# agwi-lab/renderformer

Hardware: AMD Instinct MI355X
Metric: rendered frames/sec at 512×512, renderformer-v1.1-swin-large, 1/2/4/8 MI355X (higher is better)
Workload: dtype fp16+bf16

## Files before the change

renderformer_amd/csrc/gemm.hip:

```cpp
#include <algorithm>
#include <type_traits>
#include <cmath>
#include <math.h>
#include <stdio.h>
#include <stdlib.h>
#include <string.h>

#include "common.h"
#include "env.h"

namespace {

constexpr int BK = 32;
constexpr int P_F16 = 2;

enum Epi { E_BF16 = RF_EPI_BF16, E_F32 = RF_EPI_F32, E_ADD = RF_EPI_ADD_F32, E_SWIGLU = RF_EPI_SWIGLU, E_CONV = 16,
           E_ROPE = 17 };

template <int BM_, int BN_, int WGM_, int WGN_, int STAGES_, int KH_ = 1>
struct Tile {
    static constexpr int BM = BM_, BN = BN_, WGM = WGM_, WGN = WGN_, STAGES = STAGES_, KH = KH_;
    static constexpr int NWAVE = WGM * WGN, THREADS = NWAVE * 64;
    static constexpr int MW = BM / WGM, NWD = BN / WGN, TI = MW / 16, TJ = NWD / 16;
    static constexpr int APIECES = BM / 16;
    static constexpr bool ASHARE = APIECES < NWAVE;
    static constexpr int PA = ASHARE ? 1 : BM / 16 / NWAVE, PB = BN / 16 / NWAVE;
    static constexpr int A_BYTES = BM * BK * 2, B_BYTES = BN * BK * 2;
    static_assert(PA >= 1 && PB >= 1 && (ASHARE || PA * NWAVE * 16 == BM) && PB * NWAVE * 16 == BN,
                  "tile/wave mismatch");
    static_assert(TI >= 1 && TJ >= 2 && TJ % 2 == 0, "wave tile too small");
};

struct EngineArgs {
    const bf16_t* a;
    const bf16_t* a_lo;
    int64_t lda;
    const bf16_t* w;
    const bf16_t* w_lo;
    int64_t ldw;
    int m, n, k;
    int hi, wi, cin_pad, ho, wo, kw, stride, pad;
    uint64_t cin_m, kw_m;
    const bf16_t* zero;
    void* c;
    int64_t ldc;
    const float* bias;
    const float* res1;
    const float* res2;
    bf16_t* p_hi;
    bf16_t* p_lo;
    int p_ld;
    int cout, deconv, flags, n_fin;
    int plane_f16;
    const float* w_fin;
    const float* b_fin;
    float elu_alpha;
    float* sk_part;
    int* sk_flag;
    int sk_epoch;
    int group_m;
    const int* gate;
    int halo_lg;
    int* err;
    int spin;
    uint64_t* stamps;
    const uint8_t* sa;
    const uint8_t* sw;
    int ld_sa, ld_sw;
    int persist;
    int l2pf;
    int out_f16;
    int* range;
    bf16_t* xg;
    int64_t ldxg;
    const float* norm_g;
    float* ss_out;
    int xg_f16;
    const float* rs_part;
    float rs_n, rs_eps;
    float* seg_ss;
    int seg_w, seg_n;
// ... 253 lines not shown
            else if (younger >= 1) wait_vm<GB>();
            else wait_vm<0>();
        }
    };

#pragma unroll
    for (int s = 0; s < S; ++s)
        if (s < nk) issue(kbeg + s, s);
    wait_tile(std::min(S, nk) - 1);
    __builtin_amdgcn_s_barrier();
    __builtin_amdgcn_sched_barrier(0);
    Frags f0, f1;
    load_frags(0, f0);
    auto step = [&](int kt, Frags& cur, Frags& nxt) {
        __builtin_amdgcn_s_waitcnt(0xC07F);
        if (kt + 1 < nk) {
            const int y = std::min(S - 2, nk - 2 - kt);
            wait_tile(y < 0 ? 0 : y);
        }
        __builtin_amdgcn_s_barrier();
        __builtin_amdgcn_sched_barrier(0);
        if (kt + S < nk) issue(kbeg + kt + S, kt % S);
        if (kt + 1 < nk) load_frags(kt + 1, nxt);
        mma(cur);
    };
    for (int kt = 0; kt < nk; kt += 2) {
        step(kt, f0, f1);
        if (kt + 1 < nk) step(kt + 1, f1, f0);
    }
}

RF_DEV uint32_t lds_addr(const char* p) { return (uint32_t)(uintptr_t)LDS_PTR(const char, p); }
RF_DEV float lds_ld_f32(const char* p) {
    float v;
    asm volatile("ds_read_b32 %0, %1\n\ts_waitcnt lgkmcnt(0)" : "=v"(v) : "v"(lds_addr(p)) : "memory");
    return v;
}
RF_DEV f32x4 lds_ld_f4(const char* p) {
    f32x4 v;
    asm volatile("ds_read_b128 %0, %1\n\ts_waitcnt lgkmcnt(0)" : "=v"(v) : "v"(lds_addr(p)) : "memory");
    return v;
}
RF_DEV void lds_st_f32(char* p, float v) { asm volatile("ds_write_b32 %0, %1" ::"v"(lds_addr(p)), "v"(v) : "memory"); }
RF_DEV void lds_sync() {
    __builtin_amdgcn_sched_barrier(0);
    asm volatile("s_waitcnt lgkmcnt(0)" ::: "memory");
    __builtin_amdgcn_s_barrier();
    __builtin_amdgcn_sched_barrier(0);
}

template <class C>
constexpr int ROPE_POS_BYTES = (C::BM * 9 + 63) / 64 * 256;
template <class C, int EPI>
constexpr int PN_AREA = EPI == E_ADD      ? C::BN * 4 + C::BM * C::WGN * 4
                        : EPI == E_BF16   ? C::BM * PN_SLOTS * 4 + C::BM * C::WGN * 4
                        : EPI == E_ROPE   ? C::BM * PN_SLOTS * 4 + C::BM * C::WGN * 4 + C::BN * 4 + ROPE_POS_BYTES<C> + 64 * 4
                        : EPI == E_SWIGLU ? C::BM * PN_SLOTS * 4
                                          : 0;

template <class C, int EPI>
RF_DEV void pn_issue(const EngineArgs& p, char* area, int m0, int n0) {
    const int lane = threadIdx.x & 63;
    const int wave = __builtin_amdgcn_readfirstlane(threadIdx.x >> 6);
    if constexpr (EPI == E_ADD) {
        if (p.xg && wave == 0 && n0 + 4 * lane < p.n && 4 * lane < C::BN)
            __builtin_amdgcn_global_load_lds(GLB_PTR(void, p.norm_g + n0 + 4 * lane), LDS_PTR(void, area), 16, 0, 0);
    } else if constexpr (EPI == E_BF16 || EPI == E_SWIGLU || EPI == E_ROPE) {
        if (p.rs_part) {
            static_assert(C::BM % 32 == 0, "1-KiB pieces of 32 rows");
            for (int c = wave; c < C::BM / 32; c += C::NWAVE) {
                const int row = min(m0 + 32 * c + (lane >> 1), p.m - 1);
                __builtin_amdgcn_global_load_lds(GLB_PTR(void, p.rs_part + (int64_t)row * PN_SLOTS + 4 * (lane & 1)),
                                                 LDS_PTR(void, area + c * 1024), 16, 0, 0);
            }
        }
        if constexpr (EPI == E_ROPE) {
            if (n0 / p.seg_w < p.seg_n) {
                char* const gl = area + C::BM * PN_SLOTS * 4 + C::BM * C::WGN * 4;
                char* const pl = gl + C::BN * 4;
                char* const fl = pl + ROPE_POS_BYTES<C>;
                if (wave == 0 && p.rope_g && 4 * lane < C::BN)
                    __builtin_amdgcn_global_load_lds(GLB_PTR(void, p.rope_g + n0 + 4 * lane), LDS_PTR(void, gl), 16, 0, 0);
                if (p.rope_pos) {
                    if (wave == C::NWAVE - 1)
                        __builtin_amdgcn_global_load_lds(GLB_PTR(void, p.rope_freqs + min(lane, p.rope_nf - 1)),
                                                         LDS_PTR(void, fl), 4, 0, 0);
                    for (int c = wave; c * 64 < C::BM * 9; c += C::NWAVE) {
                        const int e = c * 64 + lane;
                        const int r = e / 9, col = e - r * 9;
                        const int row = min(m0 + min(r, C::BM - 1), p.m - 1) / p.rope_div;
                        __builtin_amdgcn_global_load_lds(GLB_PTR(void, p.rope_pos + (int64_t)row * p.rope_ld + col),
                                                         LDS_PTR(void, pl + c * 256), 4, 0, 0);
                    }
                }
            }
        }
    }
}

template <class C, int EPI, int TW2D = 0, bool FINAL = true>
RF_DEV void engine_epilogue(const EngineArgs& p, int m0, int n0, const f32x4 (&acc)[C::TI][C::TJ],
                            char* area = nullptr) {
    constexpr int TI = C::TI, TJ = C::TJ;
    const int lane = threadIdx.x & 63;
    const int wave = threadIdx.x >> 6;
    const int wm = wave / C::WGN, wn = wave % C::WGN;
    static_assert(TW2D == 0 || (EPI == E_CONV && TW2D % 16 == 0 && C::MW % TW2D == 0), "2-D conv tile");
    const int rl = lane & 15, cq = 4 * (lane >> 4);
    const int rbase = m0 + wm * C::MW, cbase = n0 + wn * C::NWD;
    auto frow = [&](int i) -> int {
        if constexpr (TW2D == 0) return rbase + i * 16 + rl;
        else return m0 + (wm * (C::MW / TW2D) + (i * 16) / TW2D) * p.wo + (i * 16) % TW2D + rl;
    };
    float amax = 0.f;
    const bool rsc = (EPI == E_SWIGLU || EPI == E_BF16 || EPI == E_ROPE) && p.rs_part && area;
    if constexpr (EPI == E_SWIGLU || EPI == E_BF16 || EPI == E_ROPE) {
        if (rsc) {
            lds_sync();
            for (int t = threadIdx.x; t < C::BM; t += C::THREADS) {
                char* q = area + t * (PN_SLOTS * 4);
                const f32x4 a = lds_ld_f4(q), b = lds_ld_f4(q + 16);
                const float sum = ((a[0] + a[1]) + (a[2] + a[3])) + ((b[0] + b[1]) + (b[2] + b[3]));
                lds_st_f32(q, 1.0f / sqrtf(sum / p.rs_n + p.rs_eps));
            }
            lds_sync();
        }
    }
    auto row_scale = [&](int i) -> float {
        return rsc ? lds_ld_f32(area + (wm * C::MW + i * 16 + rl) * (PN_SLOTS * 4)) : 1.f;
    };
    if constexpr (EPI == E_SWIGLU) {
// ... 133 lines not shown
            const PixOp& o = ops[PF ? (i & 1) : 0];
            if (frow(i) >= p.m) continue;
#pragma unroll
            for (int j = 0; j < TJ; ++j) {
                const int col = cbase + j * 16 + cq;
                if (col >= nreal) continue;
                const int64_t pix = o.pix[j];
                const int co = o.co[j];
                const float bb[4] = {o.b[j].x, o.b[j].y, o.b[j].z, o.b[j].w};
                const float rr1[4] = {o.r1[j].x, o.r1[j].y, o.r1[j].z, o.r1[j].w};
                const float rr2[4] = {o.r2[j].x, o.r2[j].y, o.r2[j].z, o.r2[j].w};
                float v[4] = {acc[i][j][0], acc[i][j][1], acc[i][j][2], acc[i][j][3]};
#pragma unroll
                for (int e = 0; e < 4; ++e) {
                    v[e] = ((v[e] + bb[e]) + rr1[e]) + rr2[e];
                    if (p.flags & RF_CONV_SILU_OUT) v[e] = silu(v[e]);
                }
                if (outp)
                    *reinterpret_cast<float4*>(outp + pix * p.cout + co) = make_float4(v[0], v[1], v[2], v[3]);
                if (p.p_hi && p.plane_f16) {
                    float a[4] = {v[0], v[1], v[2], v[3]};
                    if (p.flags & RF_CONV_PLANE_SILU) {
#pragma unroll
                        for (int e = 0; e < 4; ++e) a[e] = silu(a[e]);
                    }
                    amax = amax3(amax3(amax, a[0], a[1]), a[2], a[3]);
                    *reinterpret_cast<uint2*>(p.p_hi + pix * p.p_ld + co) = make_uint2(pack_f16x2(a[0], a[1]),
                                                                                       pack_f16x2(a[2], a[3]));
                } else if (p.p_hi) {
                    uint32_t h[2], l[2];
#pragma unroll
                    for (int e = 0; e < 2; ++e) {
                        float a0 = v[2 * e], a1 = v[2 * e + 1];
                        if (p.flags & RF_CONV_PLANE_SILU) {
                            a0 = silu(a0);
                            a1 = silu(a1);
                        }
                        const bf16_t h0 = f32_to_bf16(a0), h1 = f32_to_bf16(a1);
                        h[e] = (uint32_t)h0 | ((uint32_t)h1 << 16);
                        l[e] = pack_bf16x2(a0 - bf16_to_f32(h0), a1 - bf16_to_f32(h1));
                    }
                    *reinterpret_cast<uint2*>(p.p_hi + pix * p.p_ld + co) = make_uint2(h[0], h[1]);
                    *reinterpret_cast<uint2*>(p.p_lo + pix * p.p_ld + co) = make_uint2(l[0], l[1]);
                }
            }
        }
        if (p.range && !f16_in_range(amax)) report_f16_range(p.range, RF_RANGE_CONV);
        return;
    } else {
        const bool pre = EPI == E_ADD && p.xg && area;
        const bool qkseg = EPI == E_ROPE && n0 / p.seg_w < p.seg_n;
        const bool segq = (EPI == E_BF16 || (EPI == E_ROPE && qkseg)) && p.seg_ss && area && n0 / p.seg_w < p.seg_n;
        char* const red = area + (EPI == E_ADD ? C::BN * 4 : C::BM * PN_SLOTS * 4);
        if (pre) lds_sync();
        float ssr[TI];
#pragma unroll
        for (int i = 0; i < TI; ++i) ssr[i] = 0.f;
        const char* const gl = area + C::BM * PN_SLOTS * 4 + C::BM * C::WGN * 4;
        const float* const pl = reinterpret_cast<const float*>(gl + C::BN * 4);
        float frq[EPI == E_ROPE ? TJ : 1][2];
        int pcol[EPI == E_ROPE ? TJ : 1][2];
        float sscale = 1.f;
        if constexpr (EPI == E_ROPE) {
            if (qkseg) {
                if (!rsc) lds_sync();
                sscale = n0 / p.seg_w == 0 ? p.rope_qscale : 1.f;
                const int lim = 9 * p.rope_nf;
                const float* fl = pl + ROPE_POS_BYTES<C> / 4;
#pragma unroll
                for (int j = 0; j < TJ; ++j) {
                    const int col = cbase + j * 16 + cq;
#pragma unroll
                    for (int t = 0; t < 2; ++t) {
                        const int m = ((col & 127) >> 1) + t;
                        const bool on = p.rope_pos && m < lim;
                        const int pc = on ? m / p.rope_nf : 0;
                        frq[j][t] = on ? fl[m - pc * p.rope_nf] : 0.f;
                        pcol[j][t] = pc;
                    }
                }
            }
        }
#pragma unroll
        for (int i = 0; i < TI; ++i) {
            const int row = rbase + i * 16 + rl;
            if (row >= p.m) continue;
            const float rsi = row_scale(i);
#pragma unroll
            for (int j = 0; j < TJ; ++j) {
                const int col = cbase + j * 16 + cq;
                if (col >= p.n) continue;
                float v[4] = {acc[i][j][0] * rsi, acc[i][j][1] * rsi, acc[i][j][2] * rsi, acc[i][j][3] * rsi};
                if (p.bias) {
                    const float4 b = *reinterpret_cast<const float4*>(p.bias + col);
                    v[0] += b.x;
                    v[1] += b.y;
                    v[2] += b.z;
                    v[3] += b.w;
                }
                const int64_t o = (int64_t)row * p.ldc + col;
                if constexpr (EPI == E_ROPE) {
                    if (qkseg) {
                        if (segq) ssr[i] += v[0] * v[0] + v[1] * v[1] + v[2] * v[2] + v[3] * v[3];
                        const f32x4 g = p.rope_g ? *reinterpret_cast<const f32x4*>(gl + (col - n0) * 4)
                                                 : f32x4{1.f, 1.f, 1.f, 1.f};
                        const float z0 = v[0] * g[0], z1 = v[1] * g[1], z2 = v[2] * g[2], z3 = v[3] * g[3];
                        const float* prow = pl + (wm * C::MW + i * 16 + rl) * 9;
                        float s0, c0, s1, c1;
                        __sincosf(prow[pcol[j][0]] * frq[j][0], &s0, &c0);
                        __sincosf(prow[pcol[j][1]] * frq[j][1], &s1, &c1);
                        v[0] = (z0 * c0 - z1 * s0) * sscale;
                        v[1] = (z1 * c0 + z0 * s0) * sscale;
                        v[2] = (z2 * c1 - z3 * s1) * sscale;
                        v[3] = (z3 * c1 + z2 * s1) * sscale;
                    }
                    *reinterpret_cast<uint2*>(reinterpret_cast<bf16_t*>(p.c) + o) =
                        make_uint2(pack_bf16x2(v[0], v[1]), pack_bf16x2(v[2], v[3]));
                } else if constexpr (EPI == E_BF16) {
                    amax = amax3(amax3(amax, v[0], v[1]), v[2], v[3]);
                    const uint32_t lo = pack16(p, v[0], v[1]), hi = pack16(p, v[2], v[3]);
                    *reinterpret_cast<uint2*>(reinterpret_cast<bf16_t*>(p.c) + o) = make_uint2(lo, hi);
                    if (segq) {
                        const float r0 = unpack16(p, lo & 0xffffu), r1 = unpack16(p, lo >> 16);
                        const float r2 = unpack16(p, hi & 0xffffu), r3 = unpack16(p, hi >> 16);
                        ssr[i] += r0 * r0 + r1 * r1 + r2 * r2 + r3 * r3;
                    }
                } else {
                    *reinterpret_cast<float4*>(reinterpret_cast<float*>(p.c) + o) = make_float4(v[0], v[1], v[2], v[3]);
                    if (pre) {
                        const f32x4 g = lds_ld_f4(area + (col - n0) * 4);
                        const float y0 = v[0] * g[0], y1 = v[1] * g[1], y2 = v[2] * g[2], y3 = v[3] * g[3];
                        amax = amax3(amax3(amax, y0, y1), y2, y3);
                        const uint32_t lo = p.xg_f16 ? pack_f16x2(y0, y1) : pack_bf16x2(y0, y1);
                        const uint32_t hi = p.xg_f16 ? pack_f16x2(y2, y3) : pack_bf16x2(y2, y3);
                        *reinterpret_cast<uint2*>(p.xg + (int64_t)row * p.ldxg + col) = make_uint2(lo, hi);
                        ssr[i] += v[0] * v[0] + v[1] * v[1] + v[2] * v[2] + v[3] * v[3];
                    }
                }
            }
        }
        if constexpr (EPI == E_BF16)
            if (p.range && !f16_in_range(amax)) report_f16_range(p.range, RF_RANGE_GEMM);
        if constexpr (EPI == E_ADD || EPI == E_BF16 || EPI == E_ROPE) {
            if (pre && p.xg_f16 && p.range && !f16_in_range(amax)) report_f16_range(p.range, RF_RANGE_RMSNORM);
            if (pre || segq) {
#pragma unroll
                for (int i = 0; i < TI; ++i) {
                    ssr[i] += __shfl_xor(ssr[i], 16, 64);
                    ssr[i] += __shfl_xor(ssr[i], 32, 64);
                }
                if (lane < 16) {
#pragma unroll
                    for (int i = 0; i < TI; ++i) lds_st_f32(red + (wn * C::BM + wm * C::MW + i * 16 + rl) * 4, ssr[i]);
                }
                lds_sync();
                int slot, nslots, ld;
                float* base;
                if (pre) {
                    slot = n0 / C::BN;
                    nslots = (p.n + C::BN - 1) / C::BN;
                    ld = PN_SLOTS;
                    base = p.ss_out;
                } else {
                    slot = (n0 % p.seg_w) / C::BN;
                    nslots = p.seg_w / C::BN;
                    ld = p.seg_n * PN_SLOTS;
                    base = p.seg_ss + (n0 / p.seg_w) * PN_SLOTS;
                }
                for (int t = threadIdx.x; t < C::BM; t += C::THREADS) {
                    const int row = m0 + t;
                    if (row < p.m) {
                        float s = 0.f;
#pragma unroll
                        for (int w = 0; w < C::WGN; ++w) s += lds_ld_f32(red + (w * C::BM + t) * 4);
                        float* dst = base + (int64_t)row * ld;
                        dst[slot] = s;
                        if (slot == 0)
                            for (int z = nslots; z < PN_SLOTS; ++z) dst[z] = 0.f;
                    }
                }
            }
        }
    }
}



namespace ph {
constexpr int BN = 256, BK2 = 64;
constexpr int REGION = 16384;
template <int BM>
struct Cfg {
    static constexpr int NREG = BM == 256 ? 4 : 3;
    static constexpr int NA = BM == 256 ? 2 : 1;
    static constexpr int A_IMG = BM * 128;
    static constexpr int TILE = A_IMG + 256 * 128;
    static constexpr int LDS = 2 * TILE;
    static constexpr int MI = BM / 32;
    static constexpr int GLDS = 2 * NREG;
    static constexpr int FA = BM == 256 ? 4 : BM / 32;
    static_assert(BM == 256 || BM == 128 || BM == 96 || BM == 64, "phased tile height");
};
template <int BM>
RF_DEV int region_row(int r, int j) {
    if constexpr (BM == 256) {
        switch (r) {
            case 0: return j < 64 ? j : j + 64;
            case 1: return j < 64 ? j + 64 : j + 128;
            case 2: return (j >> 5) * 64 + (j & 31);
            default: return (j >> 5) * 64 + 32 + (j & 31);
        }
    } else {
        switch (r) {
            case 0: return j;
            case 1: return (j >> 5) * 64 + (j & 31);
            default: return (j >> 5) * 64 + 32 + (j & 31);
        }
    }
}
template <int ROWS>
RF_DEV int img(int row, int kh, int ch) { return kh * (ROWS * 64) + row * 64 + ((ch ^ ((row >> 1) & 3)) << 4); }
}

template <int BM, int NTERM, bool GATHER, bool INITC = false>
RF_DEV void phased_mainloop(const EngineArgs& p, char* smem, int m0, int n0, int kbeg, int kend,
                            f32x4 (&acc)[BM / 32][4], bool pre = false) {
    using namespace ph;
    using G = Cfg<BM>;
    constexpr int NREG = G::NREG, NA = G::NA, MI = G::MI;
    static_assert(NTERM == 1 || NTERM == P_F16, "phased loop: single-term operands");
    constexpr int FA = G::FA;
    const int lane = threadIdx.x & 63;
    const int wave = threadIdx.x >> 6;
    const int wr = wave >> 2, wc = wave & 3;
    const int nk = kend - kbeg;
    const bool has_a = BM >= 128 || __builtin_amdgcn_readfirstlane(wave) < BM / 16;

    const int jrow = 16 * wave + (lane >> 2);
    int trow[NREG], grow[NREG];
    const bf16_t* src[NREG];
#pragma unroll
    for (int r = 0; r < NREG; ++r) {
        trow[r] = region_row<BM>(r, jrow);
        grow[r] = region_row<BM>(r, 16 * wave);
    }
    int am[NA], gi[NA], gy[NA], gx[NA];
#pragma unroll
    for (int r = 0; r < NA; ++r) {
        const int m = m0 + trow[r];
        am[r] = m < p.m ? m : p.m - 1;
        src[r] = p.a + (int64_t)am[r] * p.lda;
        gi[r] = gy[r] = gx[r] = 0;
        if constexpr (GATHER) {
            const int ox = am[r] % p.wo, t = am[r] / p.wo;
            gi[r] = m < p.m ? t / p.ho : -1;
            gy[r] = (t % p.ho) * p.stride - p.pad;
            gx[r] = ox * p.stride - p.pad;
        }
    }
#pragma unroll
    for (int r = NA; r < NREG; ++r) src[r] = p.w + (int64_t)(n0 + trow[r]) * p.ldw;
    const int lch = lane & 3;

    auto issue = [&](int kt, int r) {
        const bool is_a = r < NA;
        if (is_a && !has_a) return;
        char* base = smem + (kt & 1) * G::TILE + (is_a ? 0 : G::A_IMG);
#pragma unroll
        for (int kh = 0; kh < 2; ++kh) {
            const int row = trow[r];
            const int ch = lch ^ ((row >> 1) & 3);
            const int k0 = (kbeg + kt) * BK2 + kh * 32;
            const bf16_t* g = src[r] + k0 + ch * 8;
            if constexpr (GATHER) {
                if (is_a) {
                    const int tap = udiv_m(k0, p.cin_m), cb = k0 - tap * p.cin_pad;
                    const int ky = udiv_m(tap, p.kw_m), kx = tap - ky * p.kw;
                    const int iy = gy[r] + ky, ix = gx[r] + kx;
                    const bool ok = gi[r] >= 0 && iy >= 0 && iy < p.hi && ix >= 0 && ix < p.wi;
                    g = ok ? p.a + (((int64_t)gi[r] * p.hi + iy) * p.wi + ix) * p.cin_pad + cb + ch * 8 : p.zero;
                }
            }
            char* dst = base + kh * (is_a ? BM * 64 : 256 * 64) + grow[r] * 64;
            __builtin_amdgcn_global_load_lds(GLB_PTR(void, g), LDS_PTR(void, dst), 16, 0, 0);
        }
    };

    if (INITC && kbeg == 0) {
        load_c_acc<MI, 4>(p, m0 + wr * (BM / 2), n0 + wc * 64, acc);
    } else {
#pragma unroll
        for (int i = 0; i < MI; ++i)
#pragma unroll
            for (int j = 0; j < 4; ++j) acc[i][j] = f32x4{0.f, 0.f, 0.f, 0.f};
    }

    const int frow = lane & 15, fch = lane >> 4;
    bf16x8 fa[FA][2], fb0[2][2], fb1[2][2];
    auto read_a = [&](const char* buf, int mi) {
#pragma unroll
        for (int i = 0; i < FA; ++i)
#pragma unroll
            for (int s = 0; s < 2; ++s)
                fa[i][s] = *reinterpret_cast<const bf16x8*>(buf + img<BM>(wr * (BM / 2) + mi * 64 + i * 16 + frow, s, fch));
    };
    auto read_b = [&](const char* buf, int ni, bf16x8 (&fb)[2][2]) {
#pragma unroll
        for (int j = 0; j < 2; ++j)
#pragma unroll
            for (int s = 0; s < 2; ++s)
                fb[j][s] = *reinterpret_cast<const bf16x8*>(buf + G::A_IMG + img<256>(wc * 64 + ni * 32 + j * 16 + frow, s, fch));
    };
    auto mma = [&](int mi, int ni, const bf16x8 (&fb)[2][2]) {
        __builtin_amdgcn_s_setprio(1);
#pragma unroll
        for (int s = 0; s < 2; ++s)
#pragma unroll
            for (int i = 0; i < FA; ++i)
#pragma unroll
                for (int j = 0; j < 2; ++j) {
                    f32x4& c = acc[mi * FA + i][ni * 2 + j];
                    if constexpr (NTERM == P_F16)
                        c = __builtin_amdgcn_mfma_f32_16x16x32_f16(__builtin_bit_cast(f16x8, fb[j][s]),
                                                                   __builtin_bit_cast(f16x8, fa[i][s]), c, 0, 0, 0);
                    else
                        c = __builtin_amdgcn_mfma_f32_16x16x32_bf16(fb[j][s], fa[i][s], c, 0, 0, 0);
                }
        __builtin_amdgcn_s_setprio(0);
    };
    auto sync_in = [&]() {
        __builtin_amdgcn_s_waitcnt(0xC07F);
        __builtin_amdgcn_sched_barrier(0);
        __builtin_amdgcn_s_barrier();
        __builtin_amdgcn_sched_barrier(0);
    };
    auto sync_out = [&]() {
        __builtin_amdgcn_sched_barrier(0);
        __builtin_amdgcn_s_barrier();
        __builtin_amdgcn_sched_barrier(0);
    };

    constexpr int AHEAD = BM == 256 ? 8 : 4;
    if (!pre) {
#pragma unroll
        for (int r = 0; r < NREG; ++r) issue(0, r);
    }
    if (nk > 1) {
        if (!pre) {
#pragma unroll
            for (int r = 0; r < (BM == 256 ? NREG : 2); ++r) issue(1, r);
        }
        if (has_a) wait_vm<AHEAD>();
        else wait_vm<AHEAD - 2>();
    } else {
        wait_vm<0>();
    }
    __builtin_amdgcn_s_barrier();
    __builtin_amdgcn_sched_barrier(0);
    const bool late = __builtin_amdgcn_readfirstlane(threadIdx.x) >= 256;
    if (late) __builtin_amdgcn_s_barrier();
    __builtin_amdgcn_sched_barrier(0);

    for (int t = 0; t < nk; ++t) {
        const char* buf = smem + (t & 1) * G::TILE;
        const bool pf = t + 2 < nk;
        if constexpr (BM == 256) {
            read_b(buf, 0, fb0);
            read_a(buf, 0);
            sync_in();
            mma(0, 0, fb0);
            sync_out();
            read_b(buf, 1, fb1);
            if (pf) {
                issue(t + 2, 0);
                issue(t + 2, 2);
            }
            sync_in();
            mma(0, 1, fb1);
            sync_out();
            read_a(buf, 1);
            if (pf) issue(t + 2, 3);
            sync_in();
            mma(1, 1, fb1);
            sync_out();
            if (pf) {
                issue(t + 2, 1);
                wait_vm<8>();
            } else {
                wait_vm<0>();
            }
            sync_in();
            mma(1, 0, fb0);
            sync_out();
        } else {
            read_b(buf, 0, fb0);
            read_a(buf, 0);
            if (t + 1 < nk) issue(t + 1, 2);
            sync_in();
            mma(0, 0, fb0);
            sync_out();
            read_b(buf, 1, fb1);
            if (pf) {
                issue(t + 2, 0);
                issue(t + 2, 1);
                if (has_a) wait_vm<4>();
                else wait_vm<2>();
            } else {
                wait_vm<0>();
            }
            sync_in();
            mma(0, 1, fb1);
            sync_out();
        }
    }
    if (!late) __builtin_amdgcn_s_barrier();
}

template <int BM, int NTERM, bool INITC>
RF_DEV void phased3_mainloop(const EngineArgs& p, char* smem, int m0, int n0, int kbeg, int kend,
                             f32x4 (&acc)[BM / 32][4], char* touch_lds = nullptr) {
    using namespace ph;
    using G = Cfg<BM>;
    static_assert(BM <= 128, "three-buffer loop: short tiles");
    constexpr int NREG = 3, FA = G::FA;
    const int lane = threadIdx.x & 63;
    const int wave = threadIdx.x >> 6;
    const int wr = wave >> 2, wc = wave & 3;
    const int nk = kend - kbeg;
    const bool has_a = BM >= 128 || __builtin_amdgcn_readfirstlane(wave) < BM / 16;
    const int jrow = 16 * wave + (lane >> 2);
    int trow[NREG], grow[NREG];
    const bf16_t* src[NREG];
#pragma unroll
    for (int r = 0; r < NREG; ++r) {
        trow[r] = region_row<BM>(r, jrow);
        grow[r] = region_row<BM>(r, 16 * wave);
    }
    {
        const int m = m0 + trow[0];
        src[0] = p.a + (int64_t)(m < p.m ? m : p.m - 1) * p.lda;
// ... 112 lines not shown
        sync_in();
        mma(0, fb0);
        sync_out();
        read_b(buf, 1, fb1);
        if (t + 2 < nk) {
            if (l2pf) {
                if (has_a) wait_vm<8>();
                else wait_vm<6>();
            } else {
                if (has_a) wait_vm<6>();
                else wait_vm<4>();
            }
        } else {
            wait_vm<0>();
        }
        sync_in();
        mma(1, fb1);
        sync_out();
    }
    if (!late) __builtin_amdgcn_s_barrier();
}

template <int BM, int EPI, int NTERM = 1>
__global__ __launch_bounds__(512, 1) void phased3_kernel(EngineArgs p) {
    using TE = Tile<BM, 256, 2, 4, 4>;
#ifdef RF_STUDY
    __shared__ __attribute__((aligned(16))) char smem[3 * ph::Cfg<BM>::TILE + PN_AREA<TE, EPI> + 256];
#else
    __shared__ __attribute__((aligned(16))) char smem[3 * ph::Cfg<BM>::TILE + PN_AREA<TE, EPI>];
#endif
    if (gated_off(p)) return;
    const int tiles_m = (p.m + BM - 1) / BM;
    const int nwg = gridDim.x;
    const int hw = blockIdx.x;
    const int xcd = hw & 7, q = nwg >> 3, r = nwg & 7;
    const int wg = (xcd < r ? xcd * (q + 1) : r * (q + 1) + (xcd - r) * q) + (hw >> 3);
    int tm, tn;
    tile_coords(wg, tiles_m, p.n / ph::BN, p.group_m, tm, tn);
    f32x4 acc[BM / 32][4];
    char* const area = smem + 3 * ph::Cfg<BM>::TILE;
    pn_issue<TE, EPI>(p, area, tm * BM, tn * ph::BN);
#ifdef RF_STUDY
    char* const touch = area + PN_AREA<TE, EPI>;
#else
    char* const touch = nullptr;
#endif
    phased3_mainloop<BM, NTERM, EPI == E_ADD>(p, smem, tm * BM, tn * ph::BN, 0, p.k / ph::BK2, acc, touch);
    engine_epilogue<TE, EPI>(p, tm * BM, tn * ph::BN, acc, area);
}

template <int BM, int EPI, int NTERM, bool GATHER>
__global__ __launch_bounds__(512, 1) void phased_kernel(EngineArgs p) {
    using TE = Tile<BM, 256, 2, 4, 4>;
    __shared__ __attribute__((aligned(16))) char smem[ph::Cfg<BM>::LDS + PN_AREA<TE, EPI>];
    if (gated_off(p)) return;
    const int tiles_m = (p.m + BM - 1) / BM;
    const int nwg = gridDim.x;
    const int hw = blockIdx.x;
    const int xcd = hw & 7, q = nwg >> 3, r = nwg & 7;
    const int wg = (xcd < r ? xcd * (q + 1) : r * (q + 1) + (xcd - r) * q) + (hw >> 3);
    int tm, tn;
    tile_coords(wg, tiles_m, p.n / ph::BN, p.group_m, tm, tn);
    f32x4 acc[BM / 32][4];
    char* const area = smem + ph::Cfg<BM>::LDS;
    pn_issue<TE, EPI>(p, area, tm * BM, tn * ph::BN);
    phased_mainloop<BM, NTERM, GATHER, EPI == E_ADD>(p, smem, tm * BM, tn * ph::BN, 0, p.k / ph::BK2, acc);
    engine_epilogue<TE, EPI>(p, tm * BM, tn * ph::BN, acc, area);
}

RF_DEV void phased_issue01(const EngineArgs& p, char* smem, int m0, int n0, int nk) {
    using namespace ph;
    using G = Cfg<256>;
    const int lane = threadIdx.x & 63, wave = threadIdx.x >> 6;
    const int jrow = 16 * wave + (lane >> 2), lch = lane & 3;
#pragma unroll
    for (int kt = 0; kt < 2; ++kt) {
        if (kt == 1 && nk < 2) break;
#pragma unroll
        for (int r = 0; r < G::NREG; ++r) {
            const bool is_a = r < G::NA;
            const int trow = region_row<256>(r, jrow), grow = region_row<256>(r, 16 * wave);
            const bf16_t* src;
            if (is_a) {
                const int m = m0 + trow;
                src = p.a + (int64_t)(m < p.m ? m : p.m - 1) * p.lda;
            } else {
                src = p.w + (int64_t)(n0 + trow) * p.ldw;
            }
            char* base = smem + (kt & 1) * G::TILE + (is_a ? 0 : G::A_IMG);
#pragma unroll
            for (int kh = 0; kh < 2; ++kh) {
                const int ch = lch ^ ((trow >> 1) & 3);
                const bf16_t* g = src + kt * BK2 + kh * 32 + ch * 8;
                char* dst = base + kh * (256 * 64) + grow * 64;
                __builtin_amdgcn_global_load_lds(GLB_PTR(void, g), LDS_PTR(void, dst), 16, 0, 0);
            }
        }
    }
}

template <int EPI, int NTERM>
__global__ __launch_bounds__(512, 1) void phased_sk_kernel(EngineArgs p) {
    constexpr int TI = 8, TJ = 4, BM = 256, TS = BM * ph::BN;
    using TE = Tile<256, 256, 2, 4, 4>;
    __shared__ __attribute__((aligned(16))) char smem[ph::Cfg<BM>::LDS + PN_AREA<TE, EPI>];
    char* const area = smem + ph::Cfg<BM>::LDS;
// ... 1460 lines not shown
    p.sk_part = (float*)workspace;
    p.sk_flag = (int*)(p.sk_part + SK_PART_FLOATS);
    p.sk_epoch = rf::next_epoch(p.sk_flag, SK_MAX_GRID * sizeof(int), (hipStream_t)stream);
    if (p.sk_epoch == 0) return RF_ERR_LAUNCH;
    p.err = rf::device_error_word();
    p.spin = rf::spin_limit();
    p.stamps = RF_ENV_ONCE("RF_GEMM_STAMPS", 0) != 0 ? (uint64_t*)(p.sk_part + SK_PART_FLOATS - 65536) : nullptr;
    return RF_OK;
}

template <class F>
int with_epi(int epilogue, F&& f) {
    switch (epilogue) {
        case RF_EPI_BF16: return f(std::integral_constant<int, E_BF16>{});
        case RF_EPI_F32: return f(std::integral_constant<int, E_F32>{});
        case RF_EPI_ADD_F32: return f(std::integral_constant<int, E_ADD>{});
        default: return f(std::integral_constant<int, E_SWIGLU>{});
    }
}

inline void dense_args(EngineArgs& p, const void* a, int64_t lda, const void* w, int64_t ldw, int m, int n, int k,
                       void* c, int64_t ldc) {
    p.a = (const bf16_t*)a;
    p.lda = lda;
    p.w = (const bf16_t*)w;
    p.ldw = ldw;
    p.m = m;
    p.n = n;
    p.k = k;
    p.c = c;
    p.ldc = ldc;
}


int sk_grid(int m, int n, int k) {
    const bool env = rf::env_set("RF_GEMM_SK");
    int grid = 2 * 256;
    if (!env) return 0;
    if (env) {
        grid = rf::env_int("RF_GEMM_SK", 0);
        if (grid <= 0) return 0;
        grid = grid > SK_MAX_GRID ? SK_MAX_GRID : grid;
    }
    const int64_t tiles = (int64_t)((m + 127) / 128) * (n / 128);
    const int64_t rounds = (tiles + 511) / 512;
    const double eff = (double)tiles / (rounds * 512);
    if (!env && (eff >= 0.9 || tiles * (k / BK) < 8LL * grid)) return 0;
    return grid;
}

enum TileCode : int {
    TC_R128 = 128,
    TC_P256 = 256,
    TC_R64 = 642,
    TC_P64 = 643,
    TC_R64w4 = 644,
    TC_P3_64 = 645,
    TC_R64s6 = 646,
    TC_R96 = 962,
    TC_P96 = 963,
    TC_P3_96 = 964,
    TC_R96s5 = 965,
    TC_R96s6 = 966,
    TC_P128 = 1282,
    TC_P3_128 = 1283,
    TC_R128s4 = 1284,
    TC_R128s5 = 1285,
    TC_R128s6 = 1286,
    TC_R128w8s6 = 1288,
    TC_R256x128 = 2561,
    TC_R64k2 = 6423,
    TC_R64w4k2 = 6443,
    TC_R96k2 = 9623,
    TC_R128k2s3 = 12823,
    TC_R128k2s4 = 12824,
    TC_R128w8k2 = 12884,
};

int pick_cfg(int m, int n, int k, int epilogue = RF_EPI_BF16) {
    if (rf::env_set("RF_GEMM_TILE")) return rf::env_int("RF_GEMM_TILE", 0);
    const bool phased = n % 256 == 0 && k % 64 == 0 && rf::env_int("RF_GEMM_PHASED", 1) != 0;
    const double kk = k / 1024.0;
    const bool add = epilogue == RF_EPI_ADD_F32;
    auto cost = [&](int bm, int bn, int slots, double fixed, double per_k, double add_cost) {
        const int64_t tiles = (int64_t)((m + bm - 1) / bm) * (n / bn);
        const int64_t rounds = (tiles + 256 * slots - 1) / (256 * slots);
        return rounds * (fixed + per_k * kk + (add ? add_cost : 0.0));
    };
    int best = TC_R128;
    const int64_t t128 = (int64_t)((m + 127) / 128) * (n / 128);
    double best_c = t128 <= 256 ? cost(128, 128, 1, 5.5, 13.1, 5.0) : cost(128, 128, 2, 11.0, 14.0, 5.0);
    auto consider = [&](int cfg, double c) {
        if (c < best_c) {
            best_c = c;
            best = cfg;
        }
    };
    if (k % 64 == 0) consider(TC_R128w8k2, cost(128, 128, 1, 6.8, 10.9, 5.0));
    if (n % 256 == 0) consider(TC_R96, cost(96, 256, 1, 2.2, 16.5, 13.0));
    if (phased) {
        consider(TC_P256, cost(256, 256, 1, 11.0, 20.4, 5.0));
        consider(TC_P128, cost(128, 256, 1, 2.3, 18.4, 5.0));
        consider(TC_P3_96, cost(96, 256, 1, 6.0, 14.4, 5.0));
        consider(TC_P3_64, cost(64, 256, 1, 6.5, 11.8, 5.0));
    }
    return best;
}

__device__ __attribute__((aligned(16))) bf16_t g_zero_row[64];

namespace mx {
constexpr int BM = 256, BN = 256, KS = 128;
constexpr int A_DATA = BM * KS, B_DATA = BN * KS;
constexpr int STAGE = A_DATA + B_DATA + (BM + BN) * 4;
constexpr int TI = 8, TJ = 4;
typedef __attribute__((ext_vector_type(8))) int i32x8;
RF_DEV int off(int row, int ch) { return row * KS + ((ch ^ (row & 7)) << 4); }
}

template <bool INITC>
RF_DEV void mx8_mainloop(const EngineArgs& p, char* smem, int m0, int n0, int kbeg, int kend,
                         f32x4 (&acc)[mx::TI][mx::TJ]) {
    using namespace mx;
    const int lane = threadIdx.x & 63;
    const int wave = threadIdx.x >> 6;
    const int wm = wave >> 2, wn = wave & 3;
    const int nk = kend - kbeg;
    const uint8_t* A = reinterpret_cast<const uint8_t*>(p.a);
    const uint8_t* W = reinterpret_cast<const uint8_t*>(p.w);
    auto issue = [&](int kt, int buf) {
        char* st = smem + buf * STAGE;
        const int64_t k0 = (int64_t)(kbeg + kt) * KS;
#pragma unroll
        for (int i = 0; i < 8; ++i) {
            const int piece = wave * 8 + i;
            const bool is_a = piece < BM / 8;
            const int row = (is_a ? piece : piece - BM / 8) * 8 + (lane >> 3);
            const int ch = (lane & 7) ^ (row & 7);
            const uint8_t* src;
            if (is_a) {
                const int m = m0 + row;
                src = A + (int64_t)(m < p.m ? m : p.m - 1) * p.lda + k0 + ch * 16;
            } else {
                src = W + (int64_t)(n0 + row) * p.ldw + k0 + ch * 16;
            }
            __builtin_amdgcn_global_load_lds(GLB_PTR(void, src), LDS_PTR(void, st + (is_a ? 0 : A_DATA) + piece % (BM / 8) * 1024),
                                             16, 0, 0);
        }
        {
            const bool is_a = wave < BM / 64;
            const int row = (is_a ? wave : wave - BM / 64) * 64 + lane;
            const uint8_t* src;
            if (is_a) {
                const int m = m0 + row;
// ... 289 lines not shown

#ifdef RF_STUDY
int l2pf_dist() {
    return std::max(0, std::min(8, rf::env_int("RF_GEMM_L2PF", 0)));
}
#endif

template <int EPI, int BM, int NT = 1>
int launch_phased3(EngineArgs a, void* stream, const char* what) {
#ifdef RF_STUDY
    a.l2pf = l2pf_dist();
#endif
    const int tiles_m = (a.m + BM - 1) / BM, tiles_n = a.n / 256;
    const int nwg = tiles_n * tiles_m;
    a.group_m = pick_group_m(tiles_m, tiles_n, BM, 256, (nwg + 7) / 8, (int64_t)a.m * a.k * 2);
    RF_LAUNCH((phased3_kernel<BM, EPI, NT>), dim3(nwg), dim3(512), 0, (hipStream_t)stream, a);
    return rf::check_launch(what);
}

template <int EPI, int NT = 1>
int launch_phased_sk(EngineArgs a, int grid, void* stream, const char* what) {
    const int tiles_m = (a.m + 255) / 256, tiles_n = a.n / 256;
    a.group_m = pick_group_m(tiles_m, tiles_n, 256, 256, ((int64_t)tiles_m * tiles_n + 7) / 8);
    RF_LAUNCH((phased_sk_kernel<EPI, NT>), dim3(grid), dim3(512), 0, (hipStream_t)stream, a);
    return rf::check_launch(what);
}

bool use_phased(int n, int k) {
    return rf::env_int("RF_GEMM_PHASED", 1) != 0 && n % 256 == 0 && k % 64 == 0;
}

template <class C>
struct Ring {};
template <int BM>
struct Phased {};
template <int BM>
struct Phased3 {};

enum Pre { PRE_NONE = 0, PRE_N256 = 1, PRE_K64 = 2, PRE_PHASED = 4 };

bool pre_ok(int pre, const EngineArgs& p) {
    return (!(pre & PRE_N256) || p.n % 256 == 0) && (!(pre & PRE_K64) || p.k % 64 == 0) &&
           (!(pre & PRE_PHASED) || use_phased(p.n, p.k));
}

template <int CODE, class LOOP, int PRE, bool F16>
struct Row {};
template <class... R>
struct Rows {};

using TileTable = Rows<
    Row<TC_P256,        Phased<256>,                      PRE_PHASED,          true>,
    Row<TC_P128,        Phased<128>,                      PRE_PHASED,          true>,
    Row<TC_P256,        Ring<T256>,                       PRE_N256,            false>,
    Row<TC_R128s4,      Ring<Tile<128, 128, 2, 2, 4>>,    PRE_NONE,            false>,
    Row<TC_R128s5,      Ring<Tile<128, 128, 2, 2, 5>>,    PRE_NONE,            false>,
    Row<TC_R256x128,    Ring<T256x128>,                   PRE_NONE,            false>,
    Row<TC_R96,         Ring<T96x256>,                    PRE_N256,            true>,
    Row<TC_R64,         Ring<T64x256>,                    PRE_N256,            false>,
    Row<TC_P3_128,      Phased3<128>,                     PRE_PHASED,          true>,
    Row<TC_P3_96,       Phased3<96>,                      PRE_PHASED,          true>,
    Row<TC_P3_64,       Phased3<64>,                      PRE_PHASED,          true>,
    Row<TC_P96,         Phased<96>,                       PRE_PHASED,          false>,
    Row<TC_P64,         Phased<64>,                       PRE_PHASED,          false>,
    Row<TC_R64w4,       Ring<T64x256w4>,                  PRE_N256,            false>,
    Row<TC_R96s5,       Ring<T96x256s5>,                  PRE_N256,            false>,
    Row<TC_R96s6,       Ring<T96x256s6>,                  PRE_N256,            false>,
    Row<TC_R64s6,       Ring<T64x256s6>,                  PRE_N256,            false>,
    Row<TC_R128s6,      Ring<T128s6>,                     PRE_NONE,            false>,
    Row<TC_R128w8s6,    Ring<T128w8s6>,                   PRE_NONE,            false>,
    Row<TC_R128k2s3,    Ring<T128k2s3>,                   PRE_K64,             false>,
    Row<TC_R128k2s4,    Ring<T128k2s4>,                   PRE_K64,             false>,
    Row<TC_R128w8k2,    Ring<T128w8k2s4>,                 PRE_K64,             true>,
    Row<TC_R96k2,       Ring<T96x256k2>,                  PRE_K64 | PRE_N256,  false>,
    Row<TC_R64k2,       Ring<T64x256k2>,                  PRE_K64 | PRE_N256,  false>,
    Row<TC_R64w4k2,     Ring<T64x256w4k2>,                PRE_K64 | PRE_N256,  false>,
    Row<TC_R128,        Ring<T128>,                       PRE_NONE,            true>>;

template <int NT, class C>
int run_loop(Ring<C>, const EngineArgs& p, int epilogue, void* stream) {
    return with_epi(epilogue, [&](auto e) { return launch<C, decltype(e)::value, NT>(p, stream, "rf_gemm"); });
}
template <int NT, int BM>
int run_loop(Phased<BM>, const EngineArgs& p, int epilogue, void* stream) {
    return with_epi(epilogue, [&](auto e) {
        return launch_phased<decltype(e)::value, NT, false, BM>(p, stream, NT == P_F16 ? "rf_gemm_f16" : "rf_gemm_bf16");
    });
}
template <int NT, int BM>
int run_loop(Phased3<BM>, const EngineArgs& p, int epilogue, void* stream) {
    return with_epi(epilogue, [&](auto e) { return launch_phased3<decltype(e)::value, BM, NT>(p, stream, "rf_gemm"); });
}

template <int NT, int CODE, class LOOP, int PRE, bool F16>
bool try_row(Row<CODE, LOOP, PRE, F16>, int cfg, const EngineArgs& p, int epilogue, void* stream, int& rc) {
    if constexpr (NT == P_F16 && !F16) {
        return false;
    } else {
        if (cfg != CODE || !pre_ok(PRE, p)) return false;
        rc = run_loop<NT>(LOOP{}, p, epilogue, stream);
        return true;
    }
}

template <int NT, class... R>
int run_dp(Rows<R...>, int cfg, const EngineArgs& p, int epilogue, void* stream) {
// ... 192 lines not shown
    nio.rs_n = (float)norm_dim;
    nio.rs_eps = eps;
    nio.seg_ss = seg_ss;
    nio.seg_w = seg_w;
    nio.seg_n = seg_ss ? n_seg : 0;
    return gemm_bf16(a, lda, w, ldw, c, ldc, nullptr, m, n, k, epilogue, workspace, ws_bytes, stream, nullptr,
                     operand_dtype == RF_DT_F16, &nio);
}

template <class C, int NT>
static int launch_rope(EngineArgs p, void* stream) {
    return launch<C, E_ROPE, NT>(p, stream, "rf_gemm_qk_rope");
}

extern "C" int rf_gemm_qk_rope(const void* a, int64_t lda, const void* w, int64_t ldw, void* c, int64_t ldc, int m,
                               int n, int k, const float* ss, int norm_dim, float eps, float* seg_ss, int seg_w,
                               int n_seg, const float* norm_w, const float* pos, int64_t ld_pos, int pos_div,
                               const float* freqs, int n_freqs, float q_scale, int operand_dtype, void* workspace,
                               int64_t ws_bytes, void* stream) {
    (void)workspace;
    (void)ws_bytes;
    RF_REQUIRE(a && w && c, "rf_gemm_qk_rope: null pointer");
    RF_REQUIRE(m > 0 && n > 0 && k > 0, "rf_gemm_qk_rope: empty problem m=%d n=%d k=%d", m, n, k);
    RF_REQUIRE(operand_dtype == RF_DT_F16 || operand_dtype == RF_DT_BF16, "rf_gemm_qk_rope: operand_dtype");
    RF_REQUIRE(k % 64 == 0 && n % 128 == 0, "rf_gemm_qk_rope: needs K %% 64 == 0 and N %% 128 == 0");
    RF_REQUIRE(lda % 8 == 0 && ldw % 8 == 0 && lda >= k && ldw >= k && ((uintptr_t)a & 15) == 0 &&
                   ((uintptr_t)w & 15) == 0, "rf_gemm_qk_rope: operands must be 16-B aligned with lda/ldw >= K");
    RF_REQUIRE(ldc >= n && ldc % 4 == 0 && ((uintptr_t)c & 7) == 0, "rf_gemm_qk_rope: ldc too small/unaligned");
    RF_REQUIRE(seg_w > 0 && seg_w % 256 == 0 && seg_w % 128 == 0 && n_seg >= 1 && (int64_t)seg_w * n_seg <= n,
               "rf_gemm_qk_rope: the q/k segments must be whole 256-column tiles inside N");
    RF_REQUIRE(!seg_ss || (((uintptr_t)seg_ss & 15) == 0 && seg_w <= PN_SLOTS * 128),
               "rf_gemm_qk_rope: seg_ss must be 16-B aligned and seg_w <= %d", PN_SLOTS * 128);
    RF_REQUIRE(!ss || (((uintptr_t)ss & 15) == 0 && norm_dim > 0), "rf_gemm_qk_rope: ss must be 16-B aligned");
    RF_REQUIRE(!norm_w || ((uintptr_t)norm_w & 15) == 0, "rf_gemm_qk_rope: norm_w must be 16-B aligned");
    RF_REQUIRE(!pos || (freqs && n_freqs > 0 && 9 * n_freqs <= 64 && ld_pos >= 9 && pos_div >= 1),
               "rf_gemm_qk_rope: pos needs freqs with 9 * n_freqs <= 64, ld_pos >= 9 and pos_div >= 1");
    EngineArgs p{};
    dense_args(p, a, lda, w, ldw, m, n, k, c, ldc);
    p.rs_part = ss;
    p.rs_n = (float)norm_dim;
    p.rs_eps = eps;
    p.seg_ss = norm_w ? seg_ss : nullptr;
    p.seg_w = seg_w;
    p.seg_n = n_seg;
    p.rope_pos = pos;
    p.rope_ld = ld_pos;
    p.rope_div = pos ? pos_div : 1;
    p.rope_freqs = freqs;
    p.rope_nf = pos ? n_freqs : 1;
    p.rope_g = norm_w;
    p.rope_qscale = q_scale;
    const bool f16 = operand_dtype == RF_DT_F16;
    const int cfg = pick_cfg(m, n, k, RF_EPI_BF16);
    const bool t96 = n % 256 == 0 && cfg != TC_R128w8k2;
    if (t96) return f16 ? launch_rope<T96x256, P_F16>(p, stream) : launch_rope<T96x256, 1>(p, stream);
    return f16 ? launch_rope<T128w8k2s4, P_F16>(p, stream) : launch_rope<T128w8k2s4, 1>(p, stream);
}

extern "C" int rf_gemm_bf16_if(const int* flag, const void* a, int64_t lda, const void* w, int64_t ldw, void* c,
                               int64_t ldc, const float* bias, int m, int n, int k, int epilogue, void* workspace,
                               int64_t ws_bytes, void* stream) {
    RF_REQUIRE(flag, "rf_gemm_bf16_if: null flag");
    return gemm_bf16(a, lda, w, ldw, c, ldc, bias, m, n, k, epilogue, workspace, ws_bytes, stream, flag);
}

extern "C" int rf_gemm_mx8(const void* a, int64_t lda, const void* sa, int64_t ld_sa, const void* w, int64_t ldw,
                           const void* sw, int64_t ld_sw, void* c, int64_t ldc, const float* bias, int m, int n, int k,
                           int epilogue, void* stream) {
    RF_REQUIRE(a && w && sa && sw && c, "rf_gemm_mx8: null pointer");
    RF_REQUIRE(m > 0 && n > 0 && k > 0, "rf_gemm_mx8: empty problem");
    RF_REQUIRE(k % 128 == 0 && n % 256 == 0, "rf_gemm_mx8: K=%d must be a multiple of 128 and N=%d of 256", k, n);
    RF_REQUIRE(lda % 16 == 0 && ldw % 16 == 0 && lda >= k && ldw >= k, "rf_gemm_mx8: lda/ldw (bytes) >= K, 16-B aligned");
    RF_REQUIRE(ld_sa % 4 == 0 && ld_sw % 4 == 0 && ld_sa >= k / 32 && ld_sw >= k / 32,
               "rf_gemm_mx8: scale rows must hold K/32 bytes, 4-B aligned");
    RF_REQUIRE(((uintptr_t)a & 15) == 0 && ((uintptr_t)w & 15) == 0 && ((uintptr_t)sa & 3) == 0 && ((uintptr_t)sw & 3) == 0,
               "rf_gemm_mx8: operands 16-B / scales 4-B aligned");
    RF_REQUIRE(epilogue >= RF_EPI_BF16 && epilogue <= RF_EPI_SWIGLU, "rf_gemm_mx8: bad epilogue %d", epilogue);
    RF_REQUIRE(ldc >= (epilogue == RF_EPI_SWIGLU ? n / 2 : n) && ldc % 4 == 0, "rf_gemm_mx8: ldc too small/unaligned");
    EngineArgs p{};
    dense_args(p, a, lda, w, ldw, m, n, k, c, ldc);
    p.sa = (const uint8_t*)sa;
    p.sw = (const uint8_t*)sw;
    p.ld_sa = (int)ld_sa;
    p.ld_sw = (int)ld_sw;
    p.bias = bias;
    hipStream_t st = (hipStream_t)stream;
    if (RF_ENV_ONCE("RF_MX8_PLAIN", 0) == 0) {
        const int tiles_m = (m + 127) / 128, tiles_n = n / 256;
        const int nwg = tiles_m * tiles_n;
        p.group_m = pick_group_m(tiles_m, tiles_n, 128, 256, (nwg + 7) / 8, (int64_t)m * k);
        const dim3 g(nwg), b(512);
        return with_epi(epilogue, [&](auto e) {
            RF_LAUNCH((mx8_p3_kernel<decltype(e)::value>), g, b, 0, st, p);
            return rf::check_launch("rf_gemm_mx8");
        });
    }
    const int tiles_m = (m + 255) / 256, tiles_n = n / 256;
    const int nwg = tiles_m * tiles_n;
    p.group_m = pick_group_m(tiles_m, tiles_n, 256, 256, (nwg + 7) / 8, (int64_t)m * k);
    const dim3 g(nwg), b(512);
    return with_epi(epilogue, [&](auto e) {
        RF_LAUNCH((mx8_kernel<decltype(e)::value>), g, b, 0, st, p);
        return rf::check_launch("rf_gemm_mx8");
    });
}

// ... 454 lines not shown
```

Before: 90.97.

## Add 288-row phased GEMM tile with extra A region and row-packed reductions

Adds a BM=288 variant of the phased GEMM kernel. It loads an extra A region from one wave per row group and splits the A fragments unevenly across the two M halves (5+4). To fit this in LDS, the row-sum reduction scratch is stored inside the per-row norm slots, and a static assert enforces the 160 KiB limit. The tile selector gains a cost entry for P288, and the QK-RoPE GEMM can now dispatch it. The aim is more A reuse per B load, for shapes where the M dimension divides well into 288, at the cost of extra load-wait complexity and uneven fragment work.

```diff
diff --git a/renderformer_amd/csrc/gemm.hip b/renderformer_amd/csrc/gemm.hip
--- a/renderformer_amd/csrc/gemm.hip
+++ b/renderformer_amd/csrc/gemm.hip
@@ -26,7 +26,7 @@
     static constexpr bool ASHARE = APIECES < NWAVE;
     static constexpr int PA = ASHARE ? 1 : BM / 16 / NWAVE, PB = BN / 16 / NWAVE;
     static constexpr int A_BYTES = BM * BK * 2, B_BYTES = BN * BK * 2;
-    static_assert(PA >= 1 && PB >= 1 && (ASHARE || PA * NWAVE * 16 == BM) && PB * NWAVE * 16 == BN,
+    static_assert(PA >= 1 && PB >= 1 && (ASHARE || PA * NWAVE * 16 == BM || BM == 288) && PB * NWAVE * 16 == BN,
                   "tile/wave mismatch");
     static_assert(TI >= 1 && TJ >= 2 && TJ % 2 == 0, "wave tile too small");
 };
@@ -386,9 +386,13 @@
 template <class C>
 constexpr int ROPE_POS_BYTES = (C::BM * 9 + 63) / 64 * 256;
 template <class C, int EPI>
+constexpr bool RED_IN_ROWS = C::BM == 288 && (EPI == E_BF16 || EPI == E_ROPE) && C::WGN < PN_SLOTS;
+template <class C, int EPI>
+constexpr int PN_RED = RED_IN_ROWS<C, EPI> ? 0 : C::BM * C::WGN * 4;
+template <class C, int EPI>
 constexpr int PN_AREA = EPI == E_ADD      ? C::BN * 4 + C::BM * C::WGN * 4
-                        : EPI == E_BF16   ? C::BM * PN_SLOTS * 4 + C::BM * C::WGN * 4
-                        : EPI == E_ROPE   ? C::BM * PN_SLOTS * 4 + C::BM * C::WGN * 4 + C::BN * 4 + ROPE_POS_BYTES<C> + 64 * 4
+                        : EPI == E_BF16   ? C::BM * PN_SLOTS * 4 + PN_RED<C, EPI>
+                        : EPI == E_ROPE   ? C::BM * PN_SLOTS * 4 + PN_RED<C, EPI> + C::BN * 4 + ROPE_POS_BYTES<C> + 64 * 4
                         : EPI == E_SWIGLU ? C::BM * PN_SLOTS * 4
                                           : 0;
 
@@ -410,7 +414,7 @@
         }
         if constexpr (EPI == E_ROPE) {
             if (n0 / p.seg_w < p.seg_n) {
-                char* const gl = area + C::BM * PN_SLOTS * 4 + C::BM * C::WGN * 4;
+                char* const gl = area + C::BM * PN_SLOTS * 4 + PN_RED<C, EPI>;
                 char* const pl = gl + C::BN * 4;
                 char* const fl = pl + ROPE_POS_BYTES<C>;
                 if (wave == 0 && p.rope_g && 4 * lane < C::BN)
@@ -650,11 +654,15 @@
         const bool qkseg = EPI == E_ROPE && n0 / p.seg_w < p.seg_n;
         const bool segq = (EPI == E_BF16 || (EPI == E_ROPE && qkseg)) && p.seg_ss && area && n0 / p.seg_w < p.seg_n;
         char* const red = area + (EPI == E_ADD ? C::BN * 4 : C::BM * PN_SLOTS * 4);
+        auto red_at = [&](int w, int t) -> char* {
+            if constexpr (RED_IN_ROWS<C, EPI>) return area + t * (PN_SLOTS * 4) + (1 + w) * 4;
+            else return red + (w * C::BM + t) * 4;
+        };
         if (pre) lds_sync();
         float ssr[TI];
 #pragma unroll
         for (int i = 0; i < TI; ++i) ssr[i] = 0.f;
-        const char* const gl = area + C::BM * PN_SLOTS * 4 + C::BM * C::WGN * 4;
+        const char* const gl = area + C::BM * PN_SLOTS * 4 + PN_RED<C, EPI>;
         const float* const pl = reinterpret_cast<const float*>(gl + C::BN * 4);
         float frq[EPI == E_ROPE ? TJ : 1][2];
         int pcol[EPI == E_ROPE ? TJ : 1][2];
@@ -749,7 +757,7 @@
                 }
                 if (lane < 16) {
 #pragma unroll
-                    for (int i = 0; i < TI; ++i) lds_st_f32(red + (wn * C::BM + wm * C::MW + i * 16 + rl) * 4, ssr[i]);
+                    for (int i = 0; i < TI; ++i) lds_st_f32(red_at(wn, wm * C::MW + i * 16 + rl), ssr[i]);
                 }
                 lds_sync();
                 int slot, nslots, ld;
@@ -770,7 +778,7 @@
                     if (row < p.m) {
                         float s = 0.f;
 #pragma unroll
-                        for (int w = 0; w < C::WGN; ++w) s += lds_ld_f32(red + (w * C::BM + t) * 4);
+                        for (int w = 0; w < C::WGN; ++w) s += lds_ld_f32(red_at(w, t));
                         float* dst = base + (int64_t)row * ld;
                         dst[slot] = s;
                         if (slot == 0)
@@ -789,19 +797,30 @@
 constexpr int REGION = 16384;
 template <int BM>
 struct Cfg {
-    static constexpr int NREG = BM == 256 ? 4 : 3;
-    static constexpr int NA = BM == 256 ? 2 : 1;
+    static constexpr int NREG = BM >= 256 ? 4 : 3;
+    static constexpr int NA = BM >= 256 ? 2 : 1;
+    static constexpr int NX = BM == 288 ? 1 : 0;
     static constexpr int A_IMG = BM * 128;
     static constexpr int TILE = A_IMG + 256 * 128;
     static constexpr int LDS = 2 * TILE;
     static constexpr int MI = BM / 32;
     static constexpr int GLDS = 2 * NREG;
-    static constexpr int FA = BM == 256 ? 4 : BM / 32;
-    static_assert(BM == 256 || BM == 128 || BM == 96 || BM == 64, "phased tile height");
+    static constexpr int FA = BM == 288 ? 5 : BM == 256 ? 4 : BM / 32;
+    static constexpr int FA1 = BM == 288 ? 4 : BM == 256 ? 4 : 0;
+    static_assert(BM == 288 || BM == 256 || BM == 128 || BM == 96 || BM == 64, "phased tile height");
+    static_assert(BM < 256 || FA + FA1 == MI, "m0 + m1 fragments");
 };
 template <int BM>
 RF_DEV int region_row(int r, int j) {
-    if constexpr (BM == 256) {
+    if constexpr (BM == 288) {
+        switch (r) {
+            case 0: return j < 64 ? j : j + 80;
+            case 1: return j < 64 ? j + 80 : j + 160;
+            case 2: return (j >> 5) * 64 + (j & 31);
+            case 3: return (j >> 5) * 64 + 32 + (j & 31);
+            default: return (j < 64 ? 64 : 208) + (j & 15);
+        }
+    } else if constexpr (BM == 256) {
         switch (r) {
             case 0: return j < 64 ? j : j + 64;
             case 1: return j < 64 ? j + 64 : j + 128;
@@ -825,23 +844,26 @@
                             f32x4 (&acc)[BM / 32][4], bool pre = false) {
     using namespace ph;
     using G = Cfg<BM>;
-    constexpr int NREG = G::NREG, NA = G::NA, MI = G::MI;
+    constexpr int NREG = G::NREG, NA = G::NA, NX = G::NX, MI = G::MI;
     static_assert(NTERM == 1 || NTERM == P_F16, "phased loop: single-term operands");
-    constexpr int FA = G::FA;
+    static_assert(!(GATHER && NX), "gathered A: no RAX region");
+    constexpr int FA = G::FA, FA1 = G::FA1;
     const int lane = threadIdx.x & 63;
     const int wave = threadIdx.x >> 6;
     const int wr = wave >> 2, wc = wave & 3;
     const int nk = kend - kbeg;
     const bool has_a = BM >= 128 || __builtin_amdgcn_readfirstlane(wave) < BM / 16;
+    const bool has_x = NX && (__builtin_amdgcn_readfirstlane(wave) & 3) == 0;
 
     const int jrow = 16 * wave + (lane >> 2);
-    int trow[NREG], grow[NREG];
-    const bf16_t* src[NREG];
-#pragma unroll
-    for (int r = 0; r < NREG; ++r) {
+    int trow[NREG + NX], grow[NREG + NX];
+    const bf16_t* src[NREG + NX];
+#pragma unroll
+    for (int r = 0; r < NREG + NX; ++r) {
         trow[r] = region_row<BM>(r, jrow);
         grow[r] = region_row<BM>(r, 16 * wave);
     }
+    if constexpr (NX) src[NREG] = p.a + (int64_t)min(m0 + trow[NREG], p.m - 1) * p.lda;
     int am[NA], gi[NA], gy[NA], gx[NA];
 #pragma unroll
     for (int r = 0; r < NA; ++r) {
@@ -861,8 +883,9 @@
     const int lch = lane & 3;
 
     auto issue = [&](int kt, int r) {
-        const bool is_a = r < NA;
+        const bool is_a = r < NA || r >= NREG;
         if (is_a && !has_a) return;
+        if (r >= NREG && !has_x) return;
         char* base = smem + (kt & 1) * G::TILE + (is_a ? 0 : G::A_IMG);
 #pragma unroll
         for (int kh = 0; kh < 2; ++kh) {
@@ -871,7 +894,7 @@
             const int k0 = (kbeg + kt) * BK2 + kh * 32;
             const bf16_t* g = src[r] + k0 + ch * 8;
             if constexpr (GATHER) {
-                if (is_a) {
+                if (r < NA) {
                     const int tap = udiv_m(k0, p.cin_m), cb = k0 - tap * p.cin_pad;
                     const int ky = udiv_m(tap, p.kw_m), kx = tap - ky * p.kw;
                     const int iy = gy[r] + ky, ix = gx[r] + kx;
@@ -900,7 +923,8 @@
         for (int i = 0; i < FA; ++i)
 #pragma unroll
             for (int s = 0; s < 2; ++s)
-                fa[i][s] = *reinterpret_cast<const bf16x8*>(buf + img<BM>(wr * (BM / 2) + mi * 64 + i * 16 + frow, s, fch));
+                if (i < (mi ? FA1 : FA))
+                    fa[i][s] = *reinterpret_cast<const bf16x8*>(buf + img<BM>(wr * (BM / 2) + mi * (FA * 16) + i * 16 + frow, s, fch));
     };
     auto read_b = [&](const char* buf, int ni, bf16x8 (&fb)[2][2]) {
 #pragma unroll
@@ -917,6 +941,7 @@
             for (int i = 0; i < FA; ++i)
 #pragma unroll
                 for (int j = 0; j < 2; ++j) {
+                    if (i >= (mi ? FA1 : FA)) continue;
                     f32x4& c = acc[mi * FA + i][ni * 2 + j];
                     if constexpr (NTERM == P_F16)
                         c = __builtin_amdgcn_mfma_f32_16x16x32_f16(__builtin_bit_cast(f16x8, fb[j][s]),
@@ -938,17 +963,22 @@
         __builtin_amdgcn_sched_barrier(0);
     };
 
-    constexpr int AHEAD = BM == 256 ? 8 : 4;
+    constexpr int AHEAD = BM >= 256 ? 8 : 4;
+    auto wait_ahead = [&]() {
+        if (has_x) wait_vm<AHEAD + 2>();
+        else wait_vm<AHEAD>();
+    };
     if (!pre) {
 #pragma unroll
-        for (int r = 0; r < NREG; ++r) issue(0, r);
+        for (int r = 0; r < NREG + NX; ++r) issue(0, r);
     }
     if (nk > 1) {
         if (!pre) {
 #pragma unroll
-            for (int r = 0; r < (BM == 256 ? NREG : 2); ++r) issue(1, r);
-        }
-        if (has_a) wait_vm<AHEAD>();
+            for (int r = 0; r < (BM >= 256 ? NREG + NX : 2); ++r) issue(1, r);
+        }
+        if (BM >= 256) wait_ahead();
+        else if (has_a) wait_vm<AHEAD>();
         else wait_vm<AHEAD - 2>();
     } else {
         wait_vm<0>();
@@ -962,7 +992,7 @@
     for (int t = 0; t < nk; ++t) {
         const char* buf = smem + (t & 1) * G::TILE;
         const bool pf = t + 2 < nk;
-        if constexpr (BM == 256) {
+        if constexpr (BM >= 256) {
             read_b(buf, 0, fb0);
             read_a(buf, 0);
             sync_in();
@@ -971,6 +1001,7 @@
             read_b(buf, 1, fb1);
             if (pf) {
                 issue(t + 2, 0);
+                if constexpr (NX) issue(t + 2, NREG);
                 issue(t + 2, 2);
             }
             sync_in();
@@ -983,7 +1014,7 @@
             sync_out();
             if (pf) {
                 issue(t + 2, 1);
-                wait_vm<8>();
+                wait_ahead();
             } else {
                 wait_vm<0>();
             }
@@ -1202,6 +1233,7 @@
 template <int BM, int EPI, int NTERM, bool GATHER>
 __global__ __launch_bounds__(512, 1) void phased_kernel(EngineArgs p) {
     using TE = Tile<BM, 256, 2, 4, 4>;
+    static_assert(ph::Cfg<BM>::LDS + PN_AREA<TE, EPI> <= 160 * 1024, "phased tile: over the CU's 160 KiB of LDS");
     __shared__ __attribute__((aligned(16))) char smem[ph::Cfg<BM>::LDS + PN_AREA<TE, EPI>];
     if (gated_off(p)) return;
     const int tiles_m = (p.m + BM - 1) / BM;
@@ -2768,6 +2800,7 @@
 enum TileCode : int {
     TC_R128 = 128,
     TC_P256 = 256,
+    TC_P288 = 288,
     TC_R64 = 642,
     TC_P64 = 643,
     TC_R64w4 = 644,
@@ -2816,6 +2849,7 @@
     if (n % 256 == 0) consider(TC_R96, cost(96, 256, 1, 2.2, 16.5, 13.0));
     if (phased) {
         consider(TC_P256, cost(256, 256, 1, 11.0, 20.4, 5.0));
+        consider(TC_P288, cost(288, 256, 1, 22.5, 22.1, 5.0));
         consider(TC_P128, cost(128, 256, 1, 2.3, 18.4, 5.0));
         consider(TC_P3_96, cost(96, 256, 1, 6.0, 14.4, 5.0));
         consider(TC_P3_64, cost(64, 256, 1, 6.5, 11.8, 5.0));
@@ -3211,6 +3245,7 @@
 using TileTable = Rows<
     Row<TC_P256,        Phased<256>,                      PRE_PHASED,          true>,
     Row<TC_P128,        Phased<128>,                      PRE_PHASED,          true>,
+    Row<TC_P288,        Phased<288>,                      PRE_PHASED,          true>,
     Row<TC_P256,        Ring<T256>,                       PRE_N256,            false>,
     Row<TC_R128s4,      Ring<Tile<128, 128, 2, 2, 4>>,    PRE_NONE,            false>,
     Row<TC_R128s5,      Ring<Tile<128, 128, 2, 2, 5>>,    PRE_NONE,            false>,
@@ -3509,6 +3544,10 @@
     p.rope_qscale = q_scale;
     const bool f16 = operand_dtype == RF_DT_F16;
     const int cfg = pick_cfg(m, n, k, RF_EPI_BF16);
+    if (cfg == TC_P288 && use_phased(n, k)) {
+        return f16 ? launch_phased<E_ROPE, P_F16, false, 288>(p, stream, "rf_gemm_qk_rope")
+                   : launch_phased<E_ROPE, 1, false, 288>(p, stream, "rf_gemm_qk_rope");
+    }
     const bool t96 = n % 256 == 0 && cfg != TC_R128w8k2;
     if (t96) return f16 ? launch_rope<T96x256, P_F16>(p, stream) : launch_rope<T96x256, 1>(p, stream);
     return f16 ? launch_rope<T128w8k2s4, P_F16>(p, stream) : launch_rope<T128w8k2s4, 1>(p, stream);
```

Result: faster. 92.76, median of 6 (+2.0%).
